# real-stanford/garmentnets

Hardware: AMD Instinct MI355X
Metric: garments/s end-to-end predict (PointNet++ -> gridding -> UNet3D -> WNF decode -> marching cubes) (higher is better)
Workload: dtype f32 (f16x2 convs, f16x2 decoder MLPs, fp32 accumulation)

## Files before the change

### garmentnets_amd/csrc/upconv.hip

```cpp
#include "split_conv.h"

struct UpArgs {
    const float *src;
    const float *a, *d;
    const uint4 *wp;
    const float *out_scale;
    const float *act_inv;
    float *partial;
    int C1, B, Dc, Hc, Wc, Cout;
    int tiles_y, tiles_x;
};

template <int NT, bool F16>
__global__ __launch_bounds__(512, 1) void upconv_partial_kernel(UpArgs p) {
    constexpr int TZC = NT == 1 ? 2 : 1, NF = 2 * TZC, HZ = TZC + 2, HVOX = HZ * 100;
    using HL = HaloLayout<2, HZ>;
    constexpr int NIT = (HVOX * 4 + 511) / 512;
    __shared__ __attribute__((aligned(16))) unsigned char smem[2 * HL::BYTES + 2 * 384 * 4];
    float *const adl = reinterpret_cast<float *>(smem + 2 * HL::BYTES);
    const int tid = threadIdx.x, lane = tid & 63, h = lane >> 5, r = lane & 31;
    const int cls = __builtin_amdgcn_readfirstlane(tid >> 6), pz = cls >> 2, py = (cls >> 1) & 1, px = cls & 1;
    const unsigned nblk = gridDim.x, xcd = blockIdx.x & 7u, jx = blockIdx.x >> 3, qx = nblk >> 3, rx = nblk & 7u;
    const unsigned logical = (xcd < rx ? xcd * (qx + 1) : rx * (qx + 1) + (xcd - rx) * qx) + jx;
    const int ncb = p.Cout / (32 * NT);
    int tile = (int)(logical / (unsigned)ncb);
    const int cb = (int)(logical % (unsigned)ncb);
    const int tiles_z = (p.Dc + TZC - 1) / TZC;
    const int tz = tile % tiles_z; tile /= tiles_z;
    const int tx = tile % p.tiles_x; tile /= p.tiles_x;
    const int ty = tile;
    const int z0 = tz * TZC, y0 = ty * 8, x0 = tx * 8;
    const int b = blockIdx.y;
    const int nslices = p.C1 / 16;
    const int nblocks = p.Cout / 32;

    f32x16 acc[NF][NT], tot[NF][NT];
#pragma unroll
    for (int f = 0; f < NF; ++f)
#pragma unroll
        for (int u = 0; u < NT; ++u)
#pragma unroll
            for (int q = 0; q < 16; ++q) { acc[f][u][q] = 0.f; tot[f][u][q] = 0.f; }
    for (int i = tid; i < p.C1; i += 512) { adl[i] = p.a[(int64_t)b * p.C1 + i]; adl[384 + i] = p.d[(int64_t)b * p.C1 + i]; }

    const int c4 = (tid & 3) * 4;
    float4 raw[NIT];
    unsigned inb = 0;
    auto issue_rows = [&](int sl) {
        inb = 0;
#pragma unroll
        for (int it = 0; it < NIT; ++it) {
            const int idx = tid + it * 512;
            const int hv = (idx < HVOX * 4 ? idx : HVOX * 4 - 1) >> 2;
            const int hx = hv % 10, hy = (hv / 10) % 10, hz = hv / 100;
            const int gz = z0 + hz - 1, gy = y0 + hy - 1, gx = x0 + hx - 1;
            const bool in = idx < HVOX * 4 && gz >= 0 && gz < p.Dc && gy >= 0 && gy < p.Hc && gx >= 0 && gx < p.Wc;
            raw[it] = make_float4(0.f, 0.f, 0.f, 0.f);
            if (in) {
                raw[it] = *reinterpret_cast<const float4 *>(p.src + ((((int64_t)b * p.Dc + gz) * p.Hc + gy) * p.Wc + gx) * p.C1 + sl * 16 + c4);
                inb |= 1u << it;
            }
        }
    };
    auto convert_row = [&](int it, int sl, int buf) {
        const int idx = tid + it * 512;
        if (idx < HVOX * 4) {
            const int hv = idx >> 2;
            const float4 av = *reinterpret_cast<const float4 *>(adl + sl * 16 + c4);
            const float4 dv = *reinterpret_cast<const float4 *>(adl + 384 + sl * 16 + c4);
            float v0 = 0.f, v1 = 0.f, v2 = 0.f, v3 = 0.f;
            if (inb & (1u << it)) {
                v0 = __fmaf_rn(raw[it].x, av.x, dv.x);
                v1 = __fmaf_rn(raw[it].y, av.y, dv.y);
                v2 = __fmaf_rn(raw[it].z, av.z, dv.z);
                v3 = __fmaf_rn(raw[it].w, av.w, dv.w);
            }
            uint2 pl[2];
            split4<2, F16>(v0, v1, v2, v3, pl);
            unsigned char *dst = smem + buf * HL::BYTES + HL::at(hv / 100, (hv / 10) % 10, hv % 10) + c4 * 2;
            *reinterpret_cast<uint2 *>(dst) = pl[0];
            *reinterpret_cast<uint2 *>(dst + 32) = pl[1];
        }
    };

    issue_rows(0);
    __syncthreads();
#pragma unroll
    for (int it = 0; it < NIT; ++it) convert_row(it, 0, 0);
    __syncthreads();

    const int64_t bstep = (int64_t)8 * nblocks * 2 * 64;
    const uint4 *bw = p.wp + ((int64_t)cls * nblocks + cb * NT) * 2 * 64 + lane;
    uint4 bf[NT][2], nbf[NT][2], nnbf[NT][2];
#pragma unroll
    for (int u = 0; u < NT; ++u) { nbf[u][0] = bw[(u * 2 + 0) * 64]; nbf[u][1] = bw[(u * 2 + 1) * 64]; }
    bw += bstep;
#pragma unroll
    for (int u = 0; u < NT; ++u) { nnbf[u][0] = bw[(u * 2 + 0) * 64]; nnbf[u][1] = bw[(u * 2 + 1) * 64]; }
    bw += bstep;
    const int abase = HL::at(pz, (r >> 3) + py, (r & 7) + px) + 16 * h;
    constexpr int AF1 = 4 * HL::ROWP, AFZ = 10 * HL::ROWP;
    const int nsteps = nslices * 8;
    int step = 0;
    uint4 af[NF][2], naf[NF][2];
#pragma unroll
    for (int f = 0; f < NF; ++f) {
        naf[f][0] = *reinterpret_cast<const uint4 *>(smem + abase + (f >> 1) * AFZ + (f & 1) * AF1);
        naf[f][1] = *reinterpret_cast<const uint4 *>(smem + abase + (f >> 1) * AFZ + (f & 1) * AF1 + 32);
    }
    for (int s = 0; s < nslices; ++s) {
        const unsigned char *const halo = smem + (s & 1) * HL::BYTES, *const halo_n = smem + ((s + 1) & 1) * HL::BYTES;
        const bool more = s + 1 < nslices;
        if (more) issue_rows(s + 1);
#pragma unroll
        for (int tap = 0; tap < 8; ++tap, ++step) {
#pragma unroll
            for (int u = 0; u < NT; ++u) { bf[u][0] = nbf[u][0]; bf[u][1] = nbf[u][1]; nbf[u][0] = nnbf[u][0]; nbf[u][1] = nnbf[u][1]; }
#pragma unroll
            for (int f = 0; f < NF; ++f) { af[f][0] = naf[f][0]; af[f][1] = naf[f][1]; }
            if (step + 2 < nsteps) {
#pragma unroll
                for (int u = 0; u < NT; ++u) { nnbf[u][0] = bw[(u * 2 + 0) * 64]; nnbf[u][1] = bw[(u * 2 + 1) * 64]; }
                bw += bstep;
            }
            if (tap < 7) {
                const int toff = HL::at((tap + 1) >> 2, ((tap + 1) >> 1) & 1, (tap + 1) & 1);
#pragma unroll
                for (int f = 0; f < NF; ++f) {
                    naf[f][0] = *reinterpret_cast<const uint4 *>(halo + abase + toff + (f >> 1) * AFZ + (f & 1) * AF1);
                    naf[f][1] = *reinterpret_cast<const uint4 *>(halo + abase + toff + (f >> 1) * AFZ + (f & 1) * AF1 + 32);
                }
            }
#define UP_PROD(IA, IB)                                                                                                        \
            _Pragma("unroll") for (int u = 0; u < NT; ++u)                                                                     \
                _Pragma("unroll") for (int f = 0; f < NF; ++f) acc[f][u] = mfma16<F16>(af[f][IA], bf[u][IB], acc[f][u]);
            UP_PROD(1, 0)
            if (more && tap >= 2 && tap < 2 + NIT) convert_row(tap - 2, s + 1, (s + 1) & 1);
            UP_PROD(0, 1) UP_PROD(0, 0)
#undef UP_PROD
        }
#pragma unroll
        for (int f = 0; f < NF; ++f)
#pragma unroll
            for (int u = 0; u < NT; ++u)
#pragma unroll
                for (int q = 0; q < 16; ++q) { tot[f][u][q] = __fadd_rn(tot[f][u][q], acc[f][u][q]); acc[f][u][q] = 0.f; }
        __syncthreads();
        if (more) {
#pragma unroll
            for (int f = 0; f < NF; ++f) {
                naf[f][0] = *reinterpret_cast<const uint4 *>(halo_n + abase + (f >> 1) * AFZ + (f & 1) * AF1);
                naf[f][1] = *reinterpret_cast<const uint4 *>(halo_n + abase + (f >> 1) * AFZ + (f & 1) * AF1 + 32);
            }
        }
    }
    const int64_t pc = (int64_t)8 * p.Cout;
#pragma unroll
    for (int f = 0; f < NF; ++f)
#pragma unroll
        for (int u = 0; u < NT; ++u) {
            const int t = f & 1, gz = z0 + (f >> 1);
            const int n = cls * p.Cout + (cb * NT + u) * 32 + r;
            const float osc = p.act_inv ? __fmul_rn(p.out_scale[n], p.act_inv[b]) : p.out_scale[n];
            if (z0 + TZC <= p.Dc && y0 + 8 <= p.Hc && x0 + 8 <= p.Wc) {
                float *ob = p.partial + ((((int64_t)b * p.Dc + gz) * p.Hc + (y0 + t * 4)) * p.Wc + (x0 + 4 * h)) * pc + n;
                const int64_t rs = (int64_t)p.Wc * pc;
#pragma unroll
                for (int q = 0; q < 16; ++q) ob[(q >> 2) * rs + (q & 3) * pc] = __fmul_rn(tot[f][u][q], osc);
                continue;
            }
#pragma unroll
            for (int q = 0; q < 16; ++q) {
                const int i = (q & 3) + 8 * (q >> 2) + 4 * h;
                const int gy = y0 + t * 4 + (i >> 3), gx = x0 + (i & 7);
                if (gz < p.Dc && gy < p.Hc && gx < p.Wc)
                    p.partial[((((int64_t)b * p.Dc + gz) * p.Hc + gy) * p.Wc + gx) * pc + n] = __fmul_rn(tot[f][u][q], osc);
            }
        }
}

extern "C" int gn_upconv_partial(const float *src1, int C1, const float *a, const float *d, const void *wp, int mode, const float *out_scale,
                                 const float *act_inv_scale, int B, int Dc, int Hc, int Wc, int Cout, float *partial, void *stream) {
    GN_REQUIRE(B >= 0 && Dc > 0 && Hc > 0 && Wc > 0 && C1 > 0 && Cout > 0, "gn_upconv_partial: bad sizes");
    GN_REQUIRE(mode == GN_SPLIT_BF16X2 || mode == GN_SPLIT_F16X2, "gn_upconv_partial: two-plane modes only (GN_SPLIT_BF16X2 / GN_SPLIT_F16X2)");
    GN_REQUIRE(C1 % 16 == 0 && C1 <= 384 && Cout % 32 == 0, "gn_upconv_partial: channels must be multiples of 16 (in, <= 384) / 32 (out)");
    if (B == 0) return GN_OK;
    GN_REQUIRE(src1 && a && d && wp && out_scale && partial, "gn_upconv_partial: null pointer");
    UpArgs p;
    p.src = src1; p.a = a; p.d = d; p.wp = (const uint4 *)wp; p.out_scale = out_scale; p.act_inv = act_inv_scale; p.partial = partial;
    p.C1 = C1; p.B = B; p.Dc = Dc; p.Hc = Hc; p.Wc = Wc; p.Cout = Cout;
    p.tiles_y = (int)gn_cdiv(Hc, 8); p.tiles_x = (int)gn_cdiv(Wc, 8);
    hipStream_t st = gn_stream(stream);
    const bool f16 = mode == GN_SPLIT_F16X2;
    if (Cout % 64 == 0) {
        const unsigned g = (unsigned)(gn_cdiv(Dc, 1) * p.tiles_y * p.tiles_x * (Cout / 64));
        if (f16) hipLaunchKernelGGL((upconv_partial_kernel<2, true>), dim3(g, B), dim3(512), 0, st, p);
        else hipLaunchKernelGGL((upconv_partial_kernel<2, false>), dim3(g, B), dim3(512), 0, st, p);
    } else {
        const unsigned g = (unsigned)(gn_cdiv(Dc, 2) * p.tiles_y * p.tiles_x * (Cout / 32));
        if (f16) hipLaunchKernelGGL((upconv_partial_kernel<1, true>), dim3(g, B), dim3(512), 0, st, p);
        else hipLaunchKernelGGL((upconv_partial_kernel<1, false>), dim3(g, B), dim3(512), 0, st, p);
    }
    GN_LAUNCH_CHECK("gn_upconv_partial");
    return GN_OK;
}
```

Before: 153.2.

## Make upconv persistent with an LDS weight ring fed by async global-to-LDS loads

The transposed-conv partial kernel becomes persistent. Each workgroup walks a contiguous range of (channel block, batch, tile) items, with the workgroup count capped between one and four times the CU count. B-weight fragments are no longer register-prefetched; they are streamed into a per-wave LDS ring of depth 3 or 6 using direct global-to-LDS loads, with hand-tuned vmcnt waits, and activation rows are fetched with inline-asm buffer loads. The halo for the next item is staged during the last slice of the current one. This is meant to hide weight-load latency, cut launch and tail cost, and reuse the weight stream across tiles, at the price of much more LDS, fragile counter-based synchronisation and a new env-var knob.

After: 154.3 (median of 6 runs). Within noise of the previous version (+0.7%).

```diff
diff --git a/garmentnets_amd/csrc/upconv.hip b/garmentnets_amd/csrc/upconv.hip
--- a/garmentnets_amd/csrc/upconv.hip
+++ b/garmentnets_amd/csrc/upconv.hip
@@ -1,4 +1,5 @@
 #include "split_conv.h"
+#include <cstdlib>
 
 struct UpArgs {
     const float *src;
@@ -16,23 +17,40 @@
     constexpr int TZC = NT == 1 ? 2 : 1, NF = 2 * TZC, HZ = TZC + 2, HVOX = HZ * 100;
     using HL = HaloLayout<2, HZ>;
     constexpr int NIT = (HVOX * 4 + 511) / 512;
-    __shared__ __attribute__((aligned(16))) unsigned char smem[2 * HL::BYTES + 2 * 384 * 4];
-    float *const adl = reinterpret_cast<float *>(smem + 2 * HL::BYTES);
+    constexpr int PC = 2 * NT;
+    constexpr int DEPTH = NT == 1 ? 6 : 3;
+    constexpr int STEPB = PC * 1024, WRING = DEPTH * STEPB;
+    constexpr int TAB_OFF = 2 * HL::BYTES, RING_OFF = TAB_OFF + 2 * 384 * 4;
+    static_assert(RING_OFF + 8 * WRING <= 160 * 1024, "two halo buffers + a / d table + 8 waves x DEPTH steps of B fragments must fit the CU's 160 KB");
+    __shared__ __attribute__((aligned(16))) unsigned char smem[RING_OFF + 8 * WRING];
+    float *const adl = reinterpret_cast<float *>(smem + TAB_OFF);
     const int tid = threadIdx.x, lane = tid & 63, h = lane >> 5, r = lane & 31;
     const int cls = __builtin_amdgcn_readfirstlane(tid >> 6), pz = cls >> 2, py = (cls >> 1) & 1, px = cls & 1;
-    const unsigned nblk = gridDim.x, xcd = blockIdx.x & 7u, jx = blockIdx.x >> 3, qx = nblk >> 3, rx = nblk & 7u;
-    const unsigned logical = (xcd < rx ? xcd * (qx + 1) : rx * (qx + 1) + (xcd - rx) * qx) + jx;
+    const unsigned lds_ring = (unsigned)(size_t)(__attribute__((address_space(3))) unsigned char *)smem + RING_OFF + cls * WRING;
+    const unsigned char *const ring = smem + RING_OFF + cls * WRING + lane * 16;
+
     const int ncb = p.Cout / (32 * NT);
-    int tile = (int)(logical / (unsigned)ncb);
-    const int cb = (int)(logical % (unsigned)ncb);
+    const int nblocks = p.Cout / 32;
     const int tiles_z = (p.Dc + TZC - 1) / TZC;
-    const int tz = tile % tiles_z; tile /= tiles_z;
-    const int tx = tile % p.tiles_x; tile /= p.tiles_x;
-    const int ty = tile;
-    const int z0 = tz * TZC, y0 = ty * 8, x0 = tx * 8;
-    const int b = blockIdx.y;
+    const int tps = tiles_z * p.tiles_y * p.tiles_x;
     const int nslices = p.C1 / 16;
-    const int nblocks = p.Cout / 32;
+    const unsigned n_items = (unsigned)ncb * (unsigned)p.B * (unsigned)tps;
+    const unsigned nwg = gridDim.x, xcd = blockIdx.x & 7u, jx = blockIdx.x >> 3, qx = nwg >> 3, rx = nwg & 7u;
+    const unsigned chn = (xcd < rx ? xcd * (qx + 1) : rx * (qx + 1) + (xcd - rx) * qx) + jx;
+    int item = (int)((uint64_t)chn * n_items / nwg);
+    const int item_end = (int)((uint64_t)(chn + 1u) * n_items / nwg);
+    if (item >= item_end) return;
+    auto decode = [&](int it, int &b_, int &cb_, int &z0_, int &y0_, int &x0_) {
+        cb_ = it / (p.B * tps);
+        const int e = it - cb_ * (p.B * tps);
+        b_ = e / tps;
+        int tile = e - b_ * tps;
+        const int tz = tile % tiles_z; tile /= tiles_z;
+        const int tx = tile % p.tiles_x;
+        z0_ = tz * TZC; y0_ = (tile / p.tiles_x) * 8; x0_ = tx * 8;
+    };
+    int b, cb, z0, y0, x0;
+    decode(item, b, cb, z0, y0, x0);
 
     f32x16 acc[NF][NT], tot[NF][NT];
 #pragma unroll
@@ -41,28 +59,40 @@
         for (int u = 0; u < NT; ++u)
 #pragma unroll
             for (int q = 0; q < 16; ++q) { acc[f][u][q] = 0.f; tot[f][u][q] = 0.f; }
-    for (int i = tid; i < p.C1; i += 512) { adl[i] = p.a[(int64_t)b * p.C1 + i]; adl[384 + i] = p.d[(int64_t)b * p.C1 + i]; }
+    auto load_table = [&](int b_) {
+        for (int i = tid; i < p.C1; i += 512) { adl[i] = p.a[(int64_t)b_ * p.C1 + i]; adl[384 + i] = p.d[(int64_t)b_ * p.C1 + i]; }
+    };
 
     const int c4 = (tid & 3) * 4;
-    float4 raw[NIT];
-    unsigned inb = 0;
-    auto issue_rows = [&](int sl) {
+    const int64_t sample = (int64_t)p.Dc * p.Hc * p.Wc * p.C1;
+    unsigned voff[NIT], inb = 0;
+    const float *rbase = p.src;
+    auto set_rows = [&](int b_, int z0_, int y0_, int x0_) {
+        int t = threadIdx.x;
+        asm volatile("" : "+v"(t));
+        rbase = p.src + (int64_t)b_ * sample;
         inb = 0;
 #pragma unroll
         for (int it = 0; it < NIT; ++it) {
-            const int idx = tid + it * 512;
+            const int idx = t + it * 512;
             const int hv = (idx < HVOX * 4 ? idx : HVOX * 4 - 1) >> 2;
             const int hx = hv % 10, hy = (hv / 10) % 10, hz = hv / 100;
-            const int gz = z0 + hz - 1, gy = y0 + hy - 1, gx = x0 + hx - 1;
+            const int gz = z0_ + hz - 1, gy = y0_ + hy - 1, gx = x0_ + hx - 1;
             const bool in = idx < HVOX * 4 && gz >= 0 && gz < p.Dc && gy >= 0 && gy < p.Hc && gx >= 0 && gx < p.Wc;
-            raw[it] = make_float4(0.f, 0.f, 0.f, 0.f);
-            if (in) {
-                raw[it] = *reinterpret_cast<const float4 *>(p.src + ((((int64_t)b * p.Dc + gz) * p.Hc + gy) * p.Wc + gx) * p.C1 + sl * 16 + c4);
-                inb |= 1u << it;
-            }
+            voff[it] = (in ? (unsigned)((gz * p.Hc + gy) * p.Wc + gx) * (unsigned)p.C1 * 4u : 0u) + (unsigned)(t & 3) * 16u;
+            if (in) inb |= 1u << it;
+        }
+    };
+    f32x4 raw[NIT];
+    auto issue_rows = [&](int sl) {
+#pragma unroll
+        for (int it = 0; it < NIT; ++it) {
+            const unsigned vo = voff[it] + (unsigned)sl * 64u;
+            asm volatile("global_load_dwordx4 %0, %1, %2" : "=v"(raw[it]) : "v"(vo), "s"(rbase) : "memory");
         }
     };
     auto convert_row = [&](int it, int sl, int buf) {
+        asm volatile("" : "+v"(raw[it]));
         const int idx = tid + it * 512;
         if (idx < HVOX * 4) {
             const int hv = idx >> 2;
@@ -83,100 +113,177 @@
         }
     };
 
+    const int64_t bstep = (int64_t)8 * nblocks * 2 * 1024;
+    const int nsteps = nslices * 8;
+    const unsigned bvoff = (unsigned)(lane * 16);
+    const unsigned char *bg0 = nullptr, *bg = nullptr;
+    int wpos = 0;
+    unsigned wslot = 0, rslot = 0;
+    float osc0[NT];
+    auto load_ainv = [&](int b_) {
+        float v = 1.f;
+        if (p.act_inv) { v = p.act_inv[b_]; asm volatile("" : "+v"(v)); }
+        return v;
+    };
+    float ainv = load_ainv(b);
+    auto ring_issue = [&]() {
+#pragma unroll
+        for (int c = 0; c < PC; ++c) gn_glds16_s(bg + c * 1024, bvoff, lds_ring + wslot + c * 1024);
+        wslot = wslot + STEPB == WRING ? 0u : wslot + STEPB;
+        if (++wpos == nsteps) { wpos = 0; bg = bg0; } else bg += bstep;
+    };
+    auto ring_start = [&](int cb_) {
+        GN_WAIT_VM_ONLY(0);
+        bg0 = reinterpret_cast<const unsigned char *>(p.wp) + ((int64_t)cls * nblocks + cb_ * NT) * 2048;
+        bg = bg0; wpos = 0; wslot = 0; rslot = 0;
+#pragma unroll
+        for (int u = 0; u < NT; ++u) {
+            osc0[u] = p.out_scale[cls * p.Cout + (cb_ * NT + u) * 32 + r];
+            asm volatile("" : "+v"(osc0[u]));
+        }
+#pragma unroll
+        for (int i = 0; i < DEPTH - 1; ++i) ring_issue();
+    };
+#define UP_WAIT_CASE(N) case N: GN_WAIT_VM_ONLY(N); break;
+#define UP_WAIT(T)                                                                                                             \
+    do {                                                                                                                       \
+        const int nb_ = (DEPTH - 1) * PC + ((T) <= DEPTH - 1 ? NIT : 0);                                                        \
+        const int nr_ = (T) >= 2 && (T) < 2 + NIT ? (NIT - 1 - ((T) - 2)) + (T) * PC : 63;                                      \
+        switch (nb_ < nr_ ? nb_ : nr_) {                    \
+            UP_WAIT_CASE(1) UP_WAIT_CASE(2) UP_WAIT_CASE(3) UP_WAIT_CASE(4) UP_WAIT_CASE(5) UP_WAIT_CASE(6) UP_WAIT_CASE(7) UP_WAIT_CASE(8)          \
+            UP_WAIT_CASE(9) UP_WAIT_CASE(10) UP_WAIT_CASE(11) UP_WAIT_CASE(12) UP_WAIT_CASE(13) UP_WAIT_CASE(14) UP_WAIT_CASE(15) UP_WAIT_CASE(16)   \
+            default: GN_WAIT_VM_ONLY(0);                                                                                        \
+        }                                                                                                                      \
+    } while (0)
+
+    load_table(b);
+    set_rows(b, z0, y0, x0);
+    ring_start(cb);
     issue_rows(0);
+    GN_WAIT_VM_ONLY(0);
     __syncthreads();
 #pragma unroll
     for (int it = 0; it < NIT; ++it) convert_row(it, 0, 0);
     __syncthreads();
 
-    const int64_t bstep = (int64_t)8 * nblocks * 2 * 64;
-    const uint4 *bw = p.wp + ((int64_t)cls * nblocks + cb * NT) * 2 * 64 + lane;
-    uint4 bf[NT][2], nbf[NT][2], nnbf[NT][2];
-#pragma unroll
-    for (int u = 0; u < NT; ++u) { nbf[u][0] = bw[(u * 2 + 0) * 64]; nbf[u][1] = bw[(u * 2 + 1) * 64]; }
-    bw += bstep;
-#pragma unroll
-    for (int u = 0; u < NT; ++u) { nnbf[u][0] = bw[(u * 2 + 0) * 64]; nnbf[u][1] = bw[(u * 2 + 1) * 64]; }
-    bw += bstep;
     const int abase = HL::at(pz, (r >> 3) + py, (r & 7) + px) + 16 * h;
     constexpr int AF1 = 4 * HL::ROWP, AFZ = 10 * HL::ROWP;
-    const int nsteps = nslices * 8;
-    int step = 0;
+    uint4 bf[NT][2];
     uint4 af[NF][2], naf[NF][2];
 #pragma unroll
     for (int f = 0; f < NF; ++f) {
         naf[f][0] = *reinterpret_cast<const uint4 *>(smem + abase + (f >> 1) * AFZ + (f & 1) * AF1);
         naf[f][1] = *reinterpret_cast<const uint4 *>(smem + abase + (f >> 1) * AFZ + (f & 1) * AF1 + 32);
     }
-    for (int s = 0; s < nslices; ++s) {
-        const unsigned char *const halo = smem + (s & 1) * HL::BYTES, *const halo_n = smem + ((s + 1) & 1) * HL::BYTES;
-        const bool more = s + 1 < nslices;
-        if (more) issue_rows(s + 1);
-#pragma unroll
-        for (int tap = 0; tap < 8; ++tap, ++step) {
-#pragma unroll
-            for (int u = 0; u < NT; ++u) { bf[u][0] = nbf[u][0]; bf[u][1] = nbf[u][1]; nbf[u][0] = nnbf[u][0]; nbf[u][1] = nnbf[u][1]; }
-#pragma unroll
-            for (int f = 0; f < NF; ++f) { af[f][0] = naf[f][0]; af[f][1] = naf[f][1]; }
-            if (step + 2 < nsteps) {
-#pragma unroll
-                for (int u = 0; u < NT; ++u) { nnbf[u][0] = bw[(u * 2 + 0) * 64]; nnbf[u][1] = bw[(u * 2 + 1) * 64]; }
-                bw += bstep;
+    const int64_t pc = (int64_t)8 * p.Cout;
+    int par = 0;
+    for (;;) {
+        int nb = b, ncb_ = cb, nz0 = z0, ny0 = y0, nx0 = x0;
+        float nainv = ainv;
+        const bool has_next = item + 1 < item_end;
+        for (int s = 0; s < nslices; ++s, par ^= 1) {
+            const unsigned char *const halo = smem + par * HL::BYTES, *const halo_n = smem + (par ^ 1) * HL::BYTES;
+            const bool last = s + 1 == nslices;
+            const bool stage = !last || has_next;
+            const int nsl = last ? 0 : s + 1;
+            if (last && has_next) {
+                decode(item + 1, nb, ncb_, nz0, ny0, nx0);
+                if (nb != b) { load_table(nb); nainv = load_ainv(nb); __syncthreads(); }
+                set_rows(nb, nz0, ny0, nx0);
             }
-            if (tap < 7) {
-                const int toff = HL::at((tap + 1) >> 2, ((tap + 1) >> 1) & 1, (tap + 1) & 1);
+#pragma unroll
+            for (int tap = 0; tap < 8; ++tap) {
+                ring_issue();
+                if (tap == 0) issue_rows(nsl);
+                UP_WAIT(tap);
+#pragma unroll
+                for (int u = 0; u < NT; ++u) {
+                    bf[u][0] = *reinterpret_cast<const uint4 *>(ring + rslot + (u * 2 + 0) * 1024);
+                    bf[u][1] = *reinterpret_cast<const uint4 *>(ring + rslot + (u * 2 + 1) * 1024);
+                }
+                rslot = rslot + STEPB == WRING ? 0u : rslot + STEPB;
+#pragma unroll
+                for (int f = 0; f < NF; ++f) { af[f][0] = naf[f][0]; af[f][1] = naf[f][1]; }
+                if (tap < 7) {
+                    const int toff = HL::at((tap + 1) >> 2, ((tap + 1) >> 1) & 1, (tap + 1) & 1);
+#pragma unroll
+                    for (int f = 0; f < NF; ++f) {
+                        naf[f][0] = *reinterpret_cast<const uint4 *>(halo + abase + toff + (f >> 1) * AFZ + (f & 1) * AF1);
+                        naf[f][1] = *reinterpret_cast<const uint4 *>(halo + abase + toff + (f >> 1) * AFZ + (f & 1) * AF1 + 32);
+                    }
+                }
+#define UP_PROD(IA, IB)                                                                                                        \
+                _Pragma("unroll") for (int u = 0; u < NT; ++u)                                                                 \
+                    _Pragma("unroll") for (int f = 0; f < NF; ++f) acc[f][u] = mfma16<F16>(af[f][IA], bf[u][IB], acc[f][u]);
+                UP_PROD(1, 0)
+                if (stage && tap >= 2 && tap < 2 + NIT) convert_row(tap - 2, nsl, par ^ 1);
+                UP_PROD(0, 1) UP_PROD(0, 0)
+#undef UP_PROD
+            }
+#pragma unroll
+            for (int f = 0; f < NF; ++f)
+#pragma unroll
+                for (int u = 0; u < NT; ++u)
+#pragma unroll
+                    for (int q = 0; q < 16; ++q) { tot[f][u][q] = __fadd_rn(tot[f][u][q], acc[f][u][q]); acc[f][u][q] = 0.f; }
+            __syncthreads();
+            if (stage) {
 #pragma unroll
                 for (int f = 0; f < NF; ++f) {
-                    naf[f][0] = *reinterpret_cast<const uint4 *>(halo + abase + toff + (f >> 1) * AFZ + (f & 1) * AF1);
-                    naf[f][1] = *reinterpret_cast<const uint4 *>(halo + abase + toff + (f >> 1) * AFZ + (f & 1) * AF1 + 32);
+                    naf[f][0] = *reinterpret_cast<const uint4 *>(halo_n + abase + (f >> 1) * AFZ + (f & 1) * AF1);
+                    naf[f][1] = *reinterpret_cast<const uint4 *>(halo_n + abase + (f >> 1) * AFZ + (f & 1) * AF1 + 32);
                 }
             }
-#define UP_PROD(IA, IB)                                                                                                        \
-            _Pragma("unroll") for (int u = 0; u < NT; ++u)                                                                     \
-                _Pragma("unroll") for (int f = 0; f < NF; ++f) acc[f][u] = mfma16<F16>(af[f][IA], bf[u][IB], acc[f][u]);
-            UP_PROD(1, 0)
-            if (more && tap >= 2 && tap < 2 + NIT) convert_row(tap - 2, s + 1, (s + 1) & 1);
-            UP_PROD(0, 1) UP_PROD(0, 0)
-#undef UP_PROD
-        }
-#pragma unroll
-        for (int f = 0; f < NF; ++f)
-#pragma unroll
-            for (int u = 0; u < NT; ++u)
-#pragma unroll
-                for (int q = 0; q < 16; ++q) { tot[f][u][q] = __fadd_rn(tot[f][u][q], acc[f][u][q]); acc[f][u][q] = 0.f; }
-        __syncthreads();
-        if (more) {
-#pragma unroll
-            for (int f = 0; f < NF; ++f) {
-                naf[f][0] = *reinterpret_cast<const uint4 *>(halo_n + abase + (f >> 1) * AFZ + (f & 1) * AF1);
-                naf[f][1] = *reinterpret_cast<const uint4 *>(halo_n + abase + (f >> 1) * AFZ + (f & 1) * AF1 + 32);
-            }
-        }
+        }
+        {
+            int ye = y0, xe = x0;
+            asm volatile("" : "+s"(ye), "+s"(xe));
+            const bool inside = z0 + TZC <= p.Dc && ye + 8 <= p.Hc && xe + 8 <= p.Wc;
+#pragma unroll
+            for (int f = 0; f < NF; ++f)
+#pragma unroll
+                for (int u = 0; u < NT; ++u) {
+                    const int t = f & 1, gz = z0 + (f >> 1);
+                    const int n = cls * p.Cout + (cb * NT + u) * 32 + r;
+                    const float osc = p.act_inv ? __fmul_rn(osc0[u], ainv) : osc0[u];
+                    if (inside) {
+                        float *ob = p.partial + ((((int64_t)b * p.Dc + gz) * p.Hc + (ye + t * 4)) * p.Wc + (xe + 4 * h)) * pc + n;
+                        const int64_t rs = (int64_t)p.Wc * pc;
+#pragma unroll
+                        for (int q = 0; q < 16; ++q) { ob[(q >> 2) * rs + (q & 3) * pc] = __fmul_rn(tot[f][u][q], osc); tot[f][u][q] = 0.f; }
+                        continue;
+                    }
+#pragma unroll
+                    for (int q = 0; q < 16; ++q) {
+                        const int i = (q & 3) + 8 * (q >> 2) + 4 * h;
+                        const int gy = ye + t * 4 + (i >> 3), gx = xe + (i & 7);
+                        if (gz < p.Dc && gy < p.Hc && gx < p.Wc)
+                            p.partial[((((int64_t)b * p.Dc + gz) * p.Hc + gy) * p.Wc + gx) * pc + n] = __fmul_rn(tot[f][u][q], osc);
+                        tot[f][u][q] = 0.f;
+                    }
+                }
+        }
+        if (!has_next) break;
+        ++item;
+        if (ncb_ != cb) ring_start(ncb_);
+        b = nb; cb = ncb_; z0 = nz0; y0 = ny0; x0 = nx0; ainv = nainv;
     }
-    const int64_t pc = (int64_t)8 * p.Cout;
-#pragma unroll
-    for (int f = 0; f < NF; ++f)
-#pragma unroll
-        for (int u = 0; u < NT; ++u) {
-            const int t = f & 1, gz = z0 + (f >> 1);
-            const int n = cls * p.Cout + (cb * NT + u) * 32 + r;
-            const float osc = p.act_inv ? __fmul_rn(p.out_scale[n], p.act_inv[b]) : p.out_scale[n];
-            if (z0 + TZC <= p.Dc && y0 + 8 <= p.Hc && x0 + 8 <= p.Wc) {
-                float *ob = p.partial + ((((int64_t)b * p.Dc + gz) * p.Hc + (y0 + t * 4)) * p.Wc + (x0 + 4 * h)) * pc + n;
-                const int64_t rs = (int64_t)p.Wc * pc;
-#pragma unroll
-                for (int q = 0; q < 16; ++q) ob[(q >> 2) * rs + (q & 3) * pc] = __fmul_rn(tot[f][u][q], osc);
-                continue;
-            }
-#pragma unroll
-            for (int q = 0; q < 16; ++q) {
-                const int i = (q & 3) + 8 * (q >> 2) + 4 * h;
-                const int gy = y0 + t * 4 + (i >> 3), gx = x0 + (i & 7);
-                if (gz < p.Dc && gy < p.Hc && gx < p.Wc)
-                    p.partial[((((int64_t)b * p.Dc + gz) * p.Hc + gy) * p.Wc + gx) * pc + n] = __fmul_rn(tot[f][u][q], osc);
-            }
-        }
+#undef UP_WAIT
+#undef UP_WAIT_CASE
+    GN_WAIT_VM_ONLY(0);
+}
+
+static unsigned upconv_workgroups(int64_t items) {
+    static int cus = 0;
+    if (cus == 0) {
+        int dev = 0, n = 0;
+        if (hipGetDevice(&dev) != hipSuccess || hipDeviceGetAttribute(&n, hipDeviceAttributeMultiprocessorCount, dev) != hipSuccess || n <= 0) n = 256;
+        cus = n;
+    }
+    int64_t wgs = items / 8;
+    wgs = wgs < cus ? cus : wgs > 4 * (int64_t)cus ? 4 * (int64_t)cus : wgs;
+    if (const char *e = getenv("GARMENTNETS_UPCONV_WGS")) { const int cap = atoi(e); if (cap > 0 && cap < wgs) wgs = cap; }
+    return (unsigned)(wgs < items ? wgs : items);
 }
 
 extern "C" int gn_upconv_partial(const float *src1, int C1, const float *a, const float *d, const void *wp, int mode, const float *out_scale,
@@ -186,20 +293,23 @@
     GN_REQUIRE(C1 % 16 == 0 && C1 <= 384 && Cout % 32 == 0, "gn_upconv_partial: channels must be multiples of 16 (in, <= 384) / 32 (out)");
     if (B == 0) return GN_OK;
     GN_REQUIRE(src1 && a && d && wp && out_scale && partial, "gn_upconv_partial: null pointer");
+    GN_REQUIRE((int64_t)Dc * Hc * Wc * C1 * 4 < ((int64_t)1 << 32), "gn_upconv_partial: a sample of the coarse source must be smaller than 4 GiB");
     UpArgs p;
     p.src = src1; p.a = a; p.d = d; p.wp = (const uint4 *)wp; p.out_scale = out_scale; p.act_inv = act_inv_scale; p.partial = partial;
     p.C1 = C1; p.B = B; p.Dc = Dc; p.Hc = Hc; p.Wc = Wc; p.Cout = Cout;
     p.tiles_y = (int)gn_cdiv(Hc, 8); p.tiles_x = (int)gn_cdiv(Wc, 8);
     hipStream_t st = gn_stream(stream);
     const bool f16 = mode == GN_SPLIT_F16X2;
-    if (Cout % 64 == 0) {
-        const unsigned g = (unsigned)(gn_cdiv(Dc, 1) * p.tiles_y * p.tiles_x * (Cout / 64));
-        if (f16) hipLaunchKernelGGL((upconv_partial_kernel<2, true>), dim3(g, B), dim3(512), 0, st, p);
-        else hipLaunchKernelGGL((upconv_partial_kernel<2, false>), dim3(g, B), dim3(512), 0, st, p);
+    const bool wide = Cout % 64 == 0;
+    const int64_t items = gn_cdiv(Dc, wide ? 1 : 2) * p.tiles_y * p.tiles_x * (Cout / (wide ? 64 : 32)) * (int64_t)B;
+    GN_REQUIRE(items < ((int64_t)1 << 31), "gn_upconv_partial: too many tiles");
+    const unsigned g = upconv_workgroups(items);
+    if (wide) {
+        if (f16) hipLaunchKernelGGL((upconv_partial_kernel<2, true>), dim3(g), dim3(512), 0, st, p);
+        else hipLaunchKernelGGL((upconv_partial_kernel<2, false>), dim3(g), dim3(512), 0, st, p);
     } else {
-        const unsigned g = (unsigned)(gn_cdiv(Dc, 2) * p.tiles_y * p.tiles_x * (Cout / 32));
-        if (f16) hipLaunchKernelGGL((upconv_partial_kernel<1, true>), dim3(g, B), dim3(512), 0, st, p);
-        else hipLaunchKernelGGL((upconv_partial_kernel<1, false>), dim3(g, B), dim3(512), 0, st, p);
+        if (f16) hipLaunchKernelGGL((upconv_partial_kernel<1, true>), dim3(g), dim3(512), 0, st, p);
+        else hipLaunchKernelGGL((upconv_partial_kernel<1, false>), dim3(g), dim3(512), 0, st, p);
     }
     GN_LAUNCH_CHECK("gn_upconv_partial");
     return GN_OK;
```

## Stream upconv weights through an LDS ring via direct global-to-LDS loads

Applied to the files above, without the earlier changes.

Adds a RING variant of the transposed-conv partial kernel. Weight fragments are prefetched DEPTH steps ahead with global-to-LDS async loads into a per-wave LDS ring, and completion is tracked with explicit vmcnt waits, replacing the two-deep register prefetch. Halo loads now use clamped addresses unconditionally, so the vmcnt accounting stays uniform, and issue_rows runs even on the last slice. The goal is deeper latency hiding of weight loads and lower VGPR pressure. In exchange it adds LDS use, waitcnt coupling with the halo loads, and an env-var switch, which is on by default.

New measurement: 156.7 before, 156.6 after. Within noise of the previous version (-0.1%).

```diff
diff --git a/garmentnets_amd/csrc/upconv.hip b/garmentnets_amd/csrc/upconv.hip
--- a/garmentnets_amd/csrc/upconv.hip
+++ b/garmentnets_amd/csrc/upconv.hip
@@ -11,12 +11,16 @@
     int tiles_y, tiles_x;
 };
 
-template <int NT, bool F16>
+template <int NT, bool F16, bool RING>
 __global__ __launch_bounds__(512, 1) void upconv_partial_kernel(UpArgs p) {
     constexpr int TZC = NT == 1 ? 2 : 1, NF = 2 * TZC, HZ = TZC + 2, HVOX = HZ * 100;
     using HL = HaloLayout<2, HZ>;
     constexpr int NIT = (HVOX * 4 + 511) / 512;
-    __shared__ __attribute__((aligned(16))) unsigned char smem[2 * HL::BYTES + 2 * 384 * 4];
+    constexpr int DEPTH = NT == 1 ? 4 : 2, NPC = 2 * NT, SLOTB = NPC * 1024;
+    constexpr int RING_OFF = 2 * HL::BYTES + 2 * 384 * 4, RING_BYTES = RING ? 8 * DEPTH * SLOTB : 0;
+    static_assert(DEPTH >= 2 && (DEPTH - 2) * NPC < 64, "upconv ring: the wait count must fit vmcnt");
+    static_assert(RING_OFF % 16 == 0 && RING_OFF + RING_BYTES <= 163840, "upconv ring: halo buffers + table + ring exceed the 160 KB of LDS");
+    __shared__ __attribute__((aligned(16))) unsigned char smem[RING_OFF + RING_BYTES];
     float *const adl = reinterpret_cast<float *>(smem + 2 * HL::BYTES);
     const int tid = threadIdx.x, lane = tid & 63, h = lane >> 5, r = lane & 31;
     const int cls = __builtin_amdgcn_readfirstlane(tid >> 6), pz = cls >> 2, py = (cls >> 1) & 1, px = cls & 1;
@@ -55,10 +59,16 @@
             const int hx = hv % 10, hy = (hv / 10) % 10, hz = hv / 100;
             const int gz = z0 + hz - 1, gy = y0 + hy - 1, gx = x0 + hx - 1;
             const bool in = idx < HVOX * 4 && gz >= 0 && gz < p.Dc && gy >= 0 && gy < p.Hc && gx >= 0 && gx < p.Wc;
-            raw[it] = make_float4(0.f, 0.f, 0.f, 0.f);
-            if (in) {
-                raw[it] = *reinterpret_cast<const float4 *>(p.src + ((((int64_t)b * p.Dc + gz) * p.Hc + gy) * p.Wc + gx) * p.C1 + sl * 16 + c4);
-                inb |= 1u << it;
+            if constexpr (RING) {
+                const int cz = min(max(gz, 0), p.Dc - 1), cy = min(max(gy, 0), p.Hc - 1), cx = min(max(gx, 0), p.Wc - 1);
+                raw[it] = *reinterpret_cast<const float4 *>(p.src + ((((int64_t)b * p.Dc + cz) * p.Hc + cy) * p.Wc + cx) * p.C1 + sl * 16 + c4);
+                inb |= in ? 1u << it : 0u;
+            } else {
+                raw[it] = make_float4(0.f, 0.f, 0.f, 0.f);
+                if (in) {
+                    raw[it] = *reinterpret_cast<const float4 *>(p.src + ((((int64_t)b * p.Dc + gz) * p.Hc + gy) * p.Wc + gx) * p.C1 + sl * 16 + c4);
+                    inb |= 1u << it;
+                }
             }
         }
     };
@@ -90,17 +100,41 @@
     __syncthreads();
 
     const int64_t bstep = (int64_t)8 * nblocks * 2 * 64;
+    const int nsteps = nslices * 8;
     const uint4 *bw = p.wp + ((int64_t)cls * nblocks + cb * NT) * 2 * 64 + lane;
     uint4 bf[NT][2], nbf[NT][2], nnbf[NT][2];
-#pragma unroll
-    for (int u = 0; u < NT; ++u) { nbf[u][0] = bw[(u * 2 + 0) * 64]; nbf[u][1] = bw[(u * 2 + 1) * 64]; }
-    bw += bstep;
-#pragma unroll
-    for (int u = 0; u < NT; ++u) { nnbf[u][0] = bw[(u * 2 + 0) * 64]; nnbf[u][1] = bw[(u * 2 + 1) * 64]; }
-    bw += bstep;
+    const unsigned char *bws = reinterpret_cast<const unsigned char *>(p.wp + ((int64_t)cls * nblocks + cb * NT) * 2 * 64);
+    const unsigned bvoff = (unsigned)lane * 16u;
+    const unsigned ring_lds = (unsigned)(size_t)(__attribute__((address_space(3))) unsigned char *)smem + RING_OFF + cls * (DEPTH * SLOTB);
+    const unsigned char *const ring_rd = smem + RING_OFF + cls * (DEPTH * SLOTB) + lane * 16;
+    int slot = 0;
+    auto ring_issue = [&](int sl) {
+#pragma unroll
+        for (int pc = 0; pc < NPC; ++pc) gn_glds16_s(bws + pc * 1024, bvoff, ring_lds + sl * SLOTB + pc * 1024);
+        bws += bstep * 16;
+    };
+    auto ring_read = [&](int sl) {
+#pragma unroll
+        for (int u = 0; u < NT; ++u) {
+            nbf[u][0] = *reinterpret_cast<const uint4 *>(ring_rd + sl * SLOTB + (u * 2 + 0) * 1024);
+            nbf[u][1] = *reinterpret_cast<const uint4 *>(ring_rd + sl * SLOTB + (u * 2 + 1) * 1024);
+        }
+    };
+    if constexpr (RING) {
+        for (int i = 0; i < DEPTH && i < nsteps; ++i) ring_issue(i);
+        if (nsteps >= DEPTH) GN_WAIT_VM_ONLY((DEPTH - 1) * NPC); else GN_WAIT_VM_ONLY(0);
+        asm volatile("" ::: "memory");
+        ring_read(0);
+    } else {
+#pragma unroll
+        for (int u = 0; u < NT; ++u) { nbf[u][0] = bw[(u * 2 + 0) * 64]; nbf[u][1] = bw[(u * 2 + 1) * 64]; }
+        bw += bstep;
+#pragma unroll
+        for (int u = 0; u < NT; ++u) { nnbf[u][0] = bw[(u * 2 + 0) * 64]; nnbf[u][1] = bw[(u * 2 + 1) * 64]; }
+        bw += bstep;
+    }
     const int abase = HL::at(pz, (r >> 3) + py, (r & 7) + px) + 16 * h;
     constexpr int AF1 = 4 * HL::ROWP, AFZ = 10 * HL::ROWP;
-    const int nsteps = nslices * 8;
     int step = 0;
     uint4 af[NF][2], naf[NF][2];
 #pragma unroll
@@ -111,17 +145,22 @@
     for (int s = 0; s < nslices; ++s) {
         const unsigned char *const halo = smem + (s & 1) * HL::BYTES, *const halo_n = smem + ((s + 1) & 1) * HL::BYTES;
         const bool more = s + 1 < nslices;
-        if (more) issue_rows(s + 1);
+        if constexpr (RING) issue_rows(more ? s + 1 : s);
+        else if (more) issue_rows(s + 1);
 #pragma unroll
         for (int tap = 0; tap < 8; ++tap, ++step) {
 #pragma unroll
-            for (int u = 0; u < NT; ++u) { bf[u][0] = nbf[u][0]; bf[u][1] = nbf[u][1]; nbf[u][0] = nnbf[u][0]; nbf[u][1] = nnbf[u][1]; }
+            for (int u = 0; u < NT; ++u) { bf[u][0] = nbf[u][0]; bf[u][1] = nbf[u][1]; }
 #pragma unroll
             for (int f = 0; f < NF; ++f) { af[f][0] = naf[f][0]; af[f][1] = naf[f][1]; }
-            if (step + 2 < nsteps) {
-#pragma unroll
-                for (int u = 0; u < NT; ++u) { nnbf[u][0] = bw[(u * 2 + 0) * 64]; nnbf[u][1] = bw[(u * 2 + 1) * 64]; }
-                bw += bstep;
+            if constexpr (!RING) {
+#pragma unroll
+                for (int u = 0; u < NT; ++u) { nbf[u][0] = nnbf[u][0]; nbf[u][1] = nnbf[u][1]; }
+                if (step + 2 < nsteps) {
+#pragma unroll
+                    for (int u = 0; u < NT; ++u) { nnbf[u][0] = bw[(u * 2 + 0) * 64]; nnbf[u][1] = bw[(u * 2 + 1) * 64]; }
+                    bw += bstep;
+                }
             }
             if (tap < 7) {
                 const int toff = HL::at((tap + 1) >> 2, ((tap + 1) >> 1) & 1, (tap + 1) & 1);
@@ -136,6 +175,16 @@
                 _Pragma("unroll") for (int f = 0; f < NF; ++f) acc[f][u] = mfma16<F16>(af[f][IA], bf[u][IB], acc[f][u]);
             UP_PROD(1, 0)
             if (more && tap >= 2 && tap < 2 + NIT) convert_row(tap - 2, s + 1, (s + 1) & 1);
+            if constexpr (RING) {
+                const int nslot = slot + 1 == DEPTH ? 0 : slot + 1;
+                if (step + 1 < nsteps) {
+                    if (step + DEPTH <= nsteps) GN_WAIT_VM_LGKM0((DEPTH - 2) * NPC); else GN_WAIT_VM_LGKM0(0);
+                    asm volatile("" ::: "memory");
+                    ring_read(nslot);
+                }
+                if (step + DEPTH < nsteps) ring_issue(slot);
+                slot = nslot;
+            }
             UP_PROD(0, 1) UP_PROD(0, 0)
 #undef UP_PROD
         }
@@ -192,15 +241,23 @@
     p.tiles_y = (int)gn_cdiv(Hc, 8); p.tiles_x = (int)gn_cdiv(Wc, 8);
     hipStream_t st = gn_stream(stream);
     const bool f16 = mode == GN_SPLIT_F16X2;
+    bool ring = true;
+    if (const char *e = getenv("GARMENTNETS_UPCONV_RING")) ring = atoi(e) != 0;
+#define UP_LAUNCH(NT_, F16_, RING_) hipLaunchKernelGGL((upconv_partial_kernel<NT_, F16_, RING_>), dim3(g, B), dim3(512), 0, st, p)
+#define UP_LAUNCH_NT(NT_)                                                          \
+    do {                                                                           \
+        if (ring) { if (f16) UP_LAUNCH(NT_, true, true); else UP_LAUNCH(NT_, false, true); }   \
+        else { if (f16) UP_LAUNCH(NT_, true, false); else UP_LAUNCH(NT_, false, false); }      \
+    } while (0)
     if (Cout % 64 == 0) {
         const unsigned g = (unsigned)(gn_cdiv(Dc, 1) * p.tiles_y * p.tiles_x * (Cout / 64));
-        if (f16) hipLaunchKernelGGL((upconv_partial_kernel<2, true>), dim3(g, B), dim3(512), 0, st, p);
-        else hipLaunchKernelGGL((upconv_partial_kernel<2, false>), dim3(g, B), dim3(512), 0, st, p);
+        UP_LAUNCH_NT(2);
     } else {
         const unsigned g = (unsigned)(gn_cdiv(Dc, 2) * p.tiles_y * p.tiles_x * (Cout / 32));
-        if (f16) hipLaunchKernelGGL((upconv_partial_kernel<1, true>), dim3(g, B), dim3(512), 0, st, p);
-        else hipLaunchKernelGGL((upconv_partial_kernel<1, false>), dim3(g, B), dim3(512), 0, st, p);
-    }
+        UP_LAUNCH_NT(1);
+    }
+#undef UP_LAUNCH_NT
+#undef UP_LAUNCH
     GN_LAUNCH_CHECK("gn_upconv_partial");
     return GN_OK;
 }
```
